# LariWa/Fractal-Image-Compression

Hardware: NVIDIA B200
Metric: encode_evals_per_s (higher is better)
Workload: dtype u8

## Files before the change

### fractal-image-compression_b200/csrc/fic_search_umma.cu

```cuda
#include <cuda_fp16.h>

#include <cmath>
#include <mutex>
#include <tuple>
#include <vector>

#include "fic_device.cuh"

namespace fic {

namespace {

constexpr int kTileN = 128;
constexpr int kBlockM = 128;
constexpr int kAccs = 4;
constexpr int kRowsPerSB = kBlockM * kAccs;
constexpr int kEpiWarps = 16;
constexpr int kThreads = (4 + kEpiWarps) * 32;
constexpr int kChunksPerTile = kTileN / 32;
constexpr int kBoundBytes = kChunksPerTile * 2 * 4 + 16 + kChunksPerTile * 4;
constexpr int kNormOff = kChunksPerTile * 2 * 4 + 16;
constexpr int kFlagLists = 2;
constexpr int kFlagCap = 32;
constexpr float kOneMinusEps = 1.0f - 1.9073486328125e-06f;
// ... 92 lines not shown
    static constexpr int A_SB_BYTES = C::NB * A_BLOCK_BYTES;
    static constexpr int KS0 = ksplit_p0<C>();
    static constexpr int SBO_B = KS0 * 256;
    static constexpr int SBO_P1 = (C::KS_B - KS0) * 256;
    static constexpr int B_OP_BYTES = (kTileN / 8) * SBO_B;
    static constexpr int P0_BYTES = B_OP_BYTES + kBoundBytes;
    static constexpr int P1_BYTES = (kTileN / 8) * SBO_P1;
    static constexpr int B_TILE_BYTES = P0_BYTES + P1_BYTES;
    static constexpr int SLOT_BYTES = C::KSPLIT ? ((P0_BYTES + 127) / 128) * 128 : B_TILE_BYTES;
    static constexpr int PAIR_P0_BYTES = B_OP_BYTES / 2, PAIR_P1_BYTES = P1_BYTES / 2;
    static constexpr int PAIR_SLOT_BYTES = PAIR_P0_BYTES > PAIR_P1_BYTES ? PAIR_P0_BYTES : PAIR_P1_BYTES;
    static constexpr int PAIR_STAGES = (C::NSTAGE * SLOT_BYTES) / PAIR_SLOT_BYTES < 12 ? (C::NSTAGE * SLOT_BYTES) / PAIR_SLOT_BYTES : 12;
    static constexpr int BAR_BYTES = 512;
    static constexpr int SMEM_BYTES = A_SB_BYTES + C::NSTAGE * SLOT_BYTES + 1024  + BAR_BYTES  +
                                      kRowsPerSB * 4 ;
};

__device__ __noinline__ float flag_threshold(float lb, float tie_abs)
{
    const float rad = lb * lb * kOneMinusEps - tie_abs;
    return rad > 0.0f ? sqrtf(rad) : -1.0f;
}

struct RowFilter { float thresh, lbmax; int cnt; };
__device__ __noinline__ RowFilter flag_chunk(RowFilter st, float lb, float ub, float tie_abs, int2 *list, int chunk_id,
                                             uint32_t sh_lb, int share)
{
    if (st.cnt < kFlagCap) list[st.cnt] = make_int2(chunk_id, __float_as_int(ub));
    st.cnt++;
    if (lb > st.lbmax) {
        st.lbmax = lb;
        if (share)
            asm volatile("red.shared.max.u32 [%0], %1;" ::"r"(sh_lb), "r"(__float_as_uint(lb)) : "memory");
        const float rad = lb * lb * kOneMinusEps - tie_abs;
        st.thresh = rad > 0.0f ? sqrtf(rad) : -1.0f;
    }
    return st;
}


__host__ __device__ __forceinline__ int64_t sweep_to_sorted(int64_t pos, uint32_t mult, int64_t nch)
{
    const uint64_t chunk = (uint64_t)pos >> 5;
    return (int64_t)(((chunk * (uint64_t)mult) % (uint64_t)nch) * 32 + ((uint64_t)pos & 31));
}

__global__ void k_umma_sortkeys(const int32_t *__restrict__ dsum, const int32_t *__restrict__ dsq, int n,
                                int64_t ND, uint32_t *__restrict__ keys, int32_t *__restrict__ vals)
{
    int64_t j = (int64_t)blockIdx.x * blockDim.x + threadIdx.x;
    if (j >= ND) return;
    int dmean;
    keys[j] = (uint32_t)dom_var(dsum[j], dsq[j], n, &dmean);
    vals[j] = (int32_t)j;
}


constexpr int kSortSub = 512;

__global__ void __launch_bounds__(256) k_sort_hist(const uint32_t *__restrict__ keys, int64_t n, int shift, int64_t nwarps,
                                                   uint32_t *__restrict__ hist)
{
    __shared__ uint32_t s_h[8][256];
    const int warp = threadIdx.x >> 5, lane = threadIdx.x & 31;
    const int64_t gw = (int64_t)blockIdx.x * 8 + warp;
    for (int d = lane; d < 256; d += 32) s_h[warp][d] = 0;
    __syncwarp();
    if (gw < nwarps) {
        const int64_t a = gw * kSortSub, b = a + kSortSub < n ? a + kSortSub : n;
        for (int64_t i = a + lane; i < b; i += 32) atomicAdd(&s_h[warp][(keys[i] >> shift) & 255u], 1u);
        __syncwarp();
        for (int d = lane; d < 256; d += 32) hist[(int64_t)d * nwarps + gw] = s_h[warp][d];
    }
}

__global__ void __launch_bounds__(256) k_sort_scan_rows(uint32_t *__restrict__ hist, int64_t nwarps, uint32_t *__restrict__ totals)
{
// ... 95 lines not shown
__device__ __forceinline__ uint32_t pack4(int a, int b, int c, int d)
{
    return (uint32_t)(a & 0xff) | ((uint32_t)(b & 0xff) << 8) | ((uint32_t)(c & 0xff) << 16) | ((uint32_t)(d & 0xff) << 24);
}

template <int n>
__host__ __device__ __forceinline__ int64_t raw_offset(int64_t pos, int c)
{
    return (pos >> 5) * (32 * n) + c * 512 + (pos & 31) * 16;
}

__device__ __forceinline__ uint32_t pack_h2(int lo, int hi)
{
    const __half2 v = __halves2half2(__int2half_rn(lo), __int2half_rn(hi));
    return *(const uint32_t *)&v;
}

template <int B, bool F16>
__global__ void __launch_bounds__(128)
k_umma_pack_domains(const uint8_t *__restrict__ dec, const int32_t *__restrict__ dsum,
                    const int32_t *__restrict__ dsq, const int32_t *__restrict__ perm, uint8_t *__restrict__ opB,
                    int32_t *__restrict__ pos_dom, int4 *__restrict__ pos_info,
                    uint8_t *__restrict__ pos_raw, int64_t *__restrict__ dom0_pos,
                    Geom g, int64_t ntiles, uint32_t mult)
{
    using L = Lay<B, F16>;
    constexpr int n = Cfg<B, F16>::n;
    const int64_t pos = (int64_t)blockIdx.x * blockDim.x + threadIdx.x;
    const int64_t tile = pos / kTileN;
    const int row = (int)(pos % kTileN);
    const int64_t sp = sweep_to_sorted(pos, mult, ntiles * kChunksPerTile);
    constexpr bool KSPLIT = Cfg<B, F16>::KSPLIT;
    uint8_t *blob = opB + tile * L::B_TILE_BYTES;
    uint8_t *rowp = blob + (row >> 3) * L::SBO_B + (row & 7) * 16;
    uint8_t *rowp1 = blob + L::P0_BYTES + (row >> 3) * L::SBO_P1 + (row & 7) * 16;
    constexpr int NCH = L::KS0 * 2;
    constexpr int NCH1 = (Cfg<B, F16>::KS_B - L::KS0) * 2;
    float rsd_hi = 0.0f, rsd_lo = __int_as_float(0x7f800000);
    int any_l = 0;
    if (sp >= g.ND) {
#pragma unroll
        for (int c = 0; c < NCH; c++) *(uint4 *)(rowp + c * 128) = make_uint4(0, 0, 0, 0);
#pragma unroll
        for (int c = 0; c < NCH1; c++) *(uint4 *)(rowp1 + c * 128) = make_uint4(0, 0, 0, 0);
        pos_dom[pos] = -1;
        pos_info[pos] = make_int4(-1, 0, 0, 0);
    } else {
        const int64_t j = perm[sp];
        const int gx = (int)(j % g.dpw), gy = (int)(j / g.dpw);
        const uint8_t *p = dec + (int64_t)(gy * g.step) * g.sw + gx * g.step;
        int dmean;
        const int varD = dom_var(dsum[j], dsq[j], n, &dmean);
        constexpr int PCH = n / 16;
        const int sgn = (!F16 && dmean == 0) ? -1 : 1;
// ... 43 lines not shown
                        hv[e] = max(-128, min(127, dv[w * 4 + e]));
                        lv[e] = dv[w * 4 + e] - hv[e];
                        any_l |= lv[e];
                    }
                    hw[w] = pack4(hv[0], hv[1], hv[2], hv[3]);
                    lw[w] = pack4(lv[0], lv[1], lv[2], lv[3]);
                }
                *(uint4 *)(rowp + c * 128) = make_uint4(hw[0], hw[1], hw[2], hw[3]);
                if (KSPLIT) *(uint4 *)(rowp1 + c * 128) = make_uint4(lw[0], lw[1], lw[2], lw[3]);
                else *(uint4 *)(rowp + (PCH + c) * 128) = make_uint4(lw[0], lw[1], lw[2], lw[3]);
            }
        }
        if (!F16) {
            const int alpha = sgn * (dsum[j] - n * dmean);
            const int a1 = alpha / 3, a2 = (alpha - a1) / 2, a3 = alpha - a1 - a2;
            constexpr int ACH = KSPLIT ? PCH : 2 * PCH;
            *(uint4 *)(rowp + ACH * 128) = make_uint4(
                (uint32_t)((-a1) & 0xff) | ((uint32_t)((-a2) & 0xff) << 8) | ((uint32_t)((-a3) & 0xff) << 16), 0, 0, 0);
            *(uint4 *)(rowp + (ACH + 1) * 128) = make_uint4(0, 0, 0, 0);
        }
        pos_dom[pos] = (int32_t)j;
        pos_info[pos] = make_int4((int32_t)j, varD, dsum[j], 0);
        if (j == 0) *dom0_pos = pos;
        if (varD > 0) {
            float r = __double2float_rn(__ddiv_rn(1.0, __dsqrt_rn((double)varD)));
            rsd_hi = r * (1.0f + 4.76837158203125e-07f);
            rsd_lo = r * (1.0f - 4.76837158203125e-07f);
        }
    }
    for (int o = 16; o > 0; o >>= 1) {
        rsd_hi = fmaxf(rsd_hi, __shfl_xor_sync(0xffffffffu, rsd_hi, o));
        rsd_lo = fminf(rsd_lo, __shfl_xor_sync(0xffffffffu, rsd_lo, o));
    }
    if ((threadIdx.x & 31) == 0) {
        if (rsd_hi == 0.0f) rsd_lo = 0.0f;
        *(float2 *)(blob + L::B_OP_BYTES + (row >> 5) * 8) = make_float2(rsd_hi, rsd_lo);
    }
    const int tile_has_l = __syncthreads_or(any_l != 0);
    if (threadIdx.x == 0) *(uint4 *)(blob + L::B_OP_BYTES + kChunksPerTile * 8) = make_uint4((uint32_t)tile_has_l, 0, 0, 0);
}

template <int B, bool F16>
__global__ void __launch_bounds__(128)
k_umma_pack_ranges(const uint8_t *__restrict__ src, const int32_t *__restrict__ rsum, uint8_t *__restrict__ opA,
                   int32_t *__restrict__ vRout, Geom g, int64_t j0, int64_t j1, int64_t rows_padded)
{
    using L = Lay<B, F16>;
    constexpr int n = Cfg<B, F16>::n;
    int64_t i = (int64_t)blockIdx.x * blockDim.x + threadIdx.x;
    if (i >= rows_padded) return;
    int64_t sb = i / L::ROWS_SB;
    int rr = (int)(i % L::ROWS_SB);
    int blk = rr / kBlockM, row = rr % kBlockM;
    uint8_t *rowp = opA + sb * L::A_SB_BYTES + blk * L::A_BLOCK_BYTES + (row >> 3) * L::SBO_A + (row & 7) * 16;
    constexpr int NCH = Cfg<B, F16>::KS_A * 2;
    const int64_t j = j0 + i / g.n_iso;
    const int kiso = (int)(i % g.n_iso);
    if (j >= j1) {
#pragma unroll
        for (int c = 0; c < NCH; c++) *(uint4 *)(rowp + c * 128) = make_uint4(0, 0, 0, 0);
        vRout[i] = 0;
        return;
    }
    int xr = (int)(j % g.rpw), yr = (int)(j / g.rpw);
    const uint8_t *p = src + (int64_t)(yr * B) * g.W + xr * B;
    int rmean;
    vRout[i] = centred_sum(rsum[j], n, &rmean);
    constexpr int PCH = n / 16;
#pragma unroll
    for (int c = 0; c < PCH; c++) {
        uint32_t w4[4];
#pragma unroll
        for (int w = 0; w < 4; w++) {
            int k = c * 16 + w * 4;
            if (kiso == 0) {
                w4[w] = *(const uint32_t *)(p + (int64_t)(k / B) * g.W + (k % B));
            } else {
                w4[w] = 0;
#pragma unroll
                for (int e = 0; e < 4; e++) {
                    int ry, rx;
                    iso_map(iso_inverse(kiso), B, (k + e) / B, (k + e) % B, &ry, &rx);
                    w4[w] |= (uint32_t)p[(int64_t)ry * g.W + rx] << (8 * e);
                }
            }
        }
        if (F16) {
            uint32_t hw[8];
#pragma unroll
            for (int w = 0; w < 4; w++) {
// ... 334 lines not shown
    asm("dp4a.u32.u32 %0, %1, %2, %3;" : "=r"(d) : "r"(a_u8x4), "r"(b_u8x4), "r"(c));
    return d;
}

__device__ __forceinline__ uint64_t make_desc(uint32_t saddr, uint32_t lbo_bytes, uint32_t sbo_bytes)
{
    return (uint64_t)((saddr >> 4) & 0x3fff) | ((uint64_t)((lbo_bytes >> 4) & 0x3fff) << 16) |
           ((uint64_t)((sbo_bytes >> 4) & 0x3fff) << 32) | ((uint64_t)1 << 46);
}

constexpr uint32_t kIdesc = (2u << 4) | (0u << 7) | (1u << 10) | ((uint32_t)(kTileN >> 3) << 17) |
                            ((uint32_t)(kBlockM >> 4) << 24);
constexpr uint32_t kIdescF16 = (1u << 4) | (0u << 7) | (0u << 10) | ((uint32_t)(kTileN >> 3) << 17) |
                               ((uint32_t)(kBlockM >> 4) << 24);
constexpr uint32_t kIdescPair = (2u << 4) | (0u << 7) | (1u << 10) | ((uint32_t)(kTileN >> 3) << 17) |
                                ((uint32_t)((2 * kBlockM) >> 4) << 24);
constexpr uint32_t kIdescF16Pair = (1u << 4) | (0u << 7) | (0u << 10) | ((uint32_t)(kTileN >> 3) << 17) |
                                   ((uint32_t)((2 * kBlockM) >> 4) << 24);


template <int B, bool F16, bool PAIR>
__host__ __device__ constexpr int epi_of() { return (!F16 || B == 16) ? 0 : ((B == 4 || PAIR) ? 3 : 2); }

template <int B, bool F16, bool PAIR, bool DUMP>
__global__ void __launch_bounds__(kThreads, 1)
k_umma_search(const uint8_t *__restrict__ opA, const uint8_t *__restrict__ opB, const int32_t *__restrict__ vRarr,
              const float *__restrict__ nRarr, int2 *__restrict__ flag_list, int32_t *__restrict__ flag_cnt, uint32_t *__restrict__ row_lb, int n_sb,
              int n_chunks, int ntiles, int iso_shift, int64_t rows_padded, int32_t *__restrict__ dump, int64_t dump_ld, volatile int *status)
{
    using C = Cfg<B, F16>;
    using L = Lay<B, F16>;
    static_assert(!PAIR || F16 || C::KSPLIT, "CTA pairs: kind::f16, or the K-split configurations (B = 16)");
    constexpr int EPI = DUMP ? 0 : epi_of<B, F16, PAIR>();
    constexpr int NISS = (PAIR && !C::KSPLIT) ? 2 : 1;
    constexpr int NSTAGE = PAIR ? L::PAIR_STAGES : C::NSTAGE;
    constexpr int SLOT = PAIR ? L::PAIR_SLOT_BYTES : L::SLOT_BYTES;
    extern __shared__ __align__(1024) uint8_t smem_raw[];
    uint8_t *smem = (uint8_t *)(((uintptr_t)smem_raw + 1023) & ~(uintptr_t)1023);
    uint8_t *sA = smem;
    uint8_t *sB = smem + L::A_SB_BYTES;
    uint64_t *bars = (uint64_t *)(sB + C::NSTAGE * L::SLOT_BYTES);
    uint32_t bar0 = smem_u32(bars);
    asm volatile("" : "+r"(bar0));
    auto BAR_B_FULL = [&](int s) { return bar0 + 8u * s; };
    auto BAR_B_EMPTY = [&](int s) { return bar0 + 8u * (NSTAGE + s); };
    auto BAR_T_FULL = [&](int q) { return bar0 + 8u * (2 * NSTAGE + q); };
    auto BAR_T_EMPTY = [&](int q) { return bar0 + 8u * (2 * NSTAGE + kAccs + q); };
    const uint32_t BAR_A_FULL = bar0 + 8u * (2 * NSTAGE + 2 * kAccs);
    const uint32_t BAR_A_EMPTY = BAR_A_FULL + 8u;
    uint32_t *tmem_slot = (uint32_t *)(bars + 2 * NSTAGE + 2 * kAccs + 2);
    const uint32_t s_has_l = bar0 + 400u;
    uint32_t *s_lb = (uint32_t *)((uint8_t *)bars + L::BAR_BYTES);

    const int warp = threadIdx.x >> 5, lane = threadIdx.x & 31;
    const uint32_t rank = PAIR ? cluster_ctarank() : 0u;
    const int u_first = PAIR ? (int)(blockIdx.x >> 1) : (int)blockIdx.x, u_step = PAIR ? (int)(gridDim.x >> 1) : (int)gridDim.x;
    const int n_sbu = PAIR ? (n_sb >> 1) : n_sb;

    if (warp == 1 && lane == 0) {
        const uint32_t both = (PAIR && rank == 0) ? 2u : 1u;
        for (int s = 0; s < NSTAGE; s++) {
            mbar_init(BAR_B_FULL(s), both);
            mbar_init(BAR_B_EMPTY(s), NISS);
        }
        for (int q = 0; q < kAccs; q++) {
            mbar_init(BAR_T_FULL(q), 1);
            mbar_init(BAR_T_EMPTY(q), both * (kEpiWarps / kAccs));
        }
        mbar_init(BAR_A_FULL, both);
        mbar_init(BAR_A_EMPTY, NISS);
        asm volatile("fence.mbarrier_init.release.cluster;" ::: "memory");
    }
    if (warp == 2) {
        if (PAIR) {
            asm volatile("tcgen05.alloc.cta_group::2.sync.aligned.shared::cta.b32 [%0], %1;" ::"r"(smem_u32(tmem_slot)), "r"(512u) : "memory");
            asm volatile("tcgen05.relinquish_alloc_permit.cta_group::2.sync.aligned;" ::: "memory");
        } else {
            asm volatile("tcgen05.alloc.cta_group::1.sync.aligned.shared::cta.b32 [%0], %1;" ::"r"(smem_u32(tmem_slot)), "r"(512u) : "memory");
            asm volatile("tcgen05.relinquish_alloc_permit.cta_group::1.sync.aligned;" ::: "memory");
        }
    }
    tc_fence_before();
    if (PAIR) cluster_sync_all();
    else __syncthreads();
    tc_fence_after();
    const uint32_t tmem_base = *tmem_slot;

    const int n_units = n_sbu * n_chunks;

    if (warp == 0) {
        if (lane == 0) {
            uint32_t stage = 0, phase = 0, a_phase = 0;
            for (int u = u_first; u < n_units; u += u_step) {
                int sb = PAIR ? 2 * (u % n_sbu) + (int)rank : u % n_sbu, ch = u / n_sbu;
                int t0 = (int)((int64_t)ch * ntiles / n_chunks), t1 = (int)((int64_t)(ch + 1) * ntiles / n_chunks);
                mbar_wait(BAR_A_EMPTY, a_phase ^ 1, status, 1);
                mbar_expect_tx(BAR_A_FULL, L::A_SB_BYTES);
                bulk_g2s(smem_u32(sA), opA + (int64_t)sb * L::A_SB_BYTES, L::A_SB_BYTES, BAR_A_FULL);
                for (int t = t0; t < t1; t++) {
                    const uint8_t *blob = opB + (int64_t)t * L::B_TILE_BYTES;
                    if (C::KSPLIT && PAIR) {
                        const uint32_t has_l = __ldg((const uint32_t *)(blob + L::B_OP_BYTES + kChunksPerTile * 8));
                        mbar_wait(BAR_B_EMPTY(stage), phase ^ 1, status, 2);
// ... 108 lines not shown
                        for (int t = t0; t < t1; t++) {
                            mbar_wait(BAR_B_FULL(stage), phase, status, 4);
                            const uint32_t has_l = lds_volatile_u32(s_has_l + 4u * stage);
                            mbar_arrive_cluster(mapa_u32(BAR_B_FULL(stage), 0));
                            if (++stage == NSTAGE) { stage = 0; phase ^= 1; }
                            if (has_l) {
                                mbar_wait(BAR_B_FULL(stage), phase, status, 4);
                                mbar_arrive_cluster(mapa_u32(BAR_B_FULL(stage), 0));
                                if (++stage == NSTAGE) { stage = 0; phase ^= 1; }
                            }
                        }
                        a_phase ^= 1;
                    }
                }
                __syncwarp();
            }
        } else if constexpr (PAIR) {
            if (rank == 0) {
                const int qi = warp >> 1;
                uint32_t stage = 0, phase = 0, a_phase = 0, t_phase = 0;
                const uint32_t elected = elect_one();
                const uint64_t a_desc0 = make_desc(smem_u32(sA), 128, L::SBO_A);
                const uint64_t b_desc0 = make_desc(smem_u32(sB), 128, L::SBO_B);
                for (int u = u_first; u < n_units; u += u_step) {
                    int ch = u / n_sbu;
                    int t0 = (int)((int64_t)ch * ntiles / n_chunks), t1 = (int)((int64_t)(ch + 1) * ntiles / n_chunks);
                    mbar_wait(BAR_A_FULL, a_phase, status, 3);
                    for (int t = t0; t < t1; t++) {
                        mbar_wait(BAR_B_FULL(stage), phase, status, 4);
                        tc_fence_after();
                        const uint64_t b_desc = b_desc0 + (uint64_t)((stage * SLOT) >> 4);
#pragma unroll
                        for (int k = 0; k < 2; k++) {
                            const int q = qi + 2 * k;
                            mbar_wait(BAR_T_EMPTY(q), ((t_phase >> k) & 1) ^ 1, status, 5);
                            tc_fence_after();
                            if (elected) {
#pragma unroll
                                for (int s = 0; s < C::NS; s++) {
                                    const uint64_t ad = a_desc0 + (uint64_t)((q * L::A_BLOCK_BYTES + C::amap(s) * 256) >> 4);
                                    tc_mma2_f16(tmem_base + q * kTileN, ad, b_desc + (uint64_t)((s * 256) >> 4), kIdescF16Pair, s > 0 ? 1u : 0u);
                                }
                                tc_commit2(BAR_T_FULL(q), 3u);
                                if (k == 1) tc_commit2(BAR_B_EMPTY(stage), 3u);
                            }
                            __syncwarp();
                            t_phase ^= 1u << k;
                        }
                        if (++stage == NSTAGE) { stage = 0; phase ^= 1; }
                    }
                    if (elected) tc_commit2(BAR_A_EMPTY, 3u);
                    __syncwarp();
                    a_phase ^= 1;
                }
            } else if (warp == 1) {
                if (lane == 0) {
                    uint32_t stage = 0, phase = 0, a_phase = 0;
                    const uint32_t ra_full = mapa_u32(BAR_A_FULL, 0);
                    for (int u = u_first; u < n_units; u += u_step) {
                        int ch = u / n_sbu;
                        int t0 = (int)((int64_t)ch * ntiles / n_chunks), t1 = (int)((int64_t)(ch + 1) * ntiles / n_chunks);
                        mbar_wait(BAR_A_FULL, a_phase, status, 3);
                        mbar_arrive_cluster(ra_full);
                        for (int t = t0; t < t1; t++) {
// ... 95 lines not shown
    } else if (warp >= 4) {
        const int e = warp - 4;
        const int lq = e & 3, q = e >> 2;
        const uint32_t ta = tmem_base + ((uint32_t)(lq * 32) << 16) + q * kTileN;
        uint32_t tf_phase = 0;
        const uint32_t bar_hand_back = PAIR ? mapa_u32(BAR_T_EMPTY(q), 0) : BAR_T_EMPTY(q);
        auto hand_back = [&]() {
            if (PAIR) mbar_arrive_cluster(bar_hand_back);
            else mbar_arrive(bar_hand_back);
        };
        constexpr bool SLACK = B == 16 && F16;
        const int n_units_mine = q < C::NB ? n_units : 0;
        for (int u = u_first; u < n_units_mine; u += u_step) {
            int sb = PAIR ? 2 * (u % n_sbu) + (int)rank : u % n_sbu, ch = u / n_sbu;
            int t0 = (int)((int64_t)ch * ntiles / n_chunks), t1 = (int)((int64_t)(ch + 1) * ntiles / n_chunks);
            const int64_t row = (int64_t)sb * L::ROWS_SB + q * kBlockM + lq * 32 + lane;
            const int vR = vRarr[row];
            const float nR = SLACK ? nRarr[row] : 0.0f;
            RowFilter st;
            st.thresh = (vR == 0) ? __int_as_float(0x7f800000) : -1.0f;
            st.lbmax = 0.0f;
            st.cnt = 0;
            const float tie_abs = (float)(vR * vR) * 4.76837158203125e-07f;
            const uint32_t sh_lb = smem_u32(s_lb + q * kBlockM + (((lq * 32 + lane) >> iso_shift) << iso_shift));
            if (iso_shift) {
                sts_u32(sh_lb, 0u);
                __syncwarp();
            }
            if (ch > 0 && vR != 0) {
                const float seed = __uint_as_float(*(volatile const uint32_t *)(row_lb + ((row >> iso_shift) << iso_shift)));
                if (seed > 0.0f) {
                    st.lbmax = seed;
                    st.thresh = flag_threshold(seed, tie_abs);
                }
            }
            int2 *const list0 = flag_list + (((int64_t)ch * rows_padded + row) * kFlagLists) * kFlagCap;
            int cnt0 = 0, cnt1 = 0;
            for (int t = t0; t < t1; t++) {
                const float4 *gb = (const float4 *)(opB + (int64_t)t * L::B_TILE_BYTES + L::B_OP_BYTES);
                const float4 bnd01 = __ldg(gb), bnd23 = __ldg(gb + 1);
                float4 bndn = make_float4(0.0f, 0.0f, 0.0f, 0.0f);
                if (SLACK) bndn = __ldg(gb + 3);
                mbar_wait(BAR_T_FULL(q), tf_phase, status, 7);
                tc_fence_after();
                if (iso_shift) {
                    const float other = __uint_as_float(lds_volatile_u32(sh_lb));
// ... 102 lines not shown
                        }
                    }
                    const float rhi = c == 0 ? bnd01.x : (c == 1 ? bnd01.z : (c == 2 ? bnd23.x : bnd23.z));
                    const float rlo = c == 0 ? bnd01.y : (c == 1 ? bnd01.w : (c == 2 ? bnd23.y : bnd23.w));
                    float Mu = M, Ml = M;
                    if (SLACK) {
                        const float pn = nR * (c == 0 ? bndn.x : (c == 1 ? bndn.y : (c == 2 ? bndn.z : bndn.w)));
                        if (pn >= 16777216.0f) {
                            const float sl = pn * 6.0e-5f;
                            Mu = M + sl;
                            Ml = fmaxf(M - sl, 0.0f);
                        }
                    }
                    const float ub = Mu * rhi;
                    if (ub > st.thresh) {
                        st.cnt = c < 2 ? cnt0 : cnt1;
                        st = flag_chunk(st, Ml * rlo, ub, tie_abs, list0 + (c >> 1) * kFlagCap, t * kChunksPerTile + c, sh_lb, iso_shift ? 1 : 0);
                        if (c < 2) cnt0 = st.cnt;
                        else cnt1 = st.cnt;
                    }
                }
                }
                tf_phase ^= 1;
            }
            flag_cnt[((int64_t)ch * rows_padded + row) * 2] = cnt0;
            flag_cnt[((int64_t)ch * rows_padded + row) * 2 + 1] = cnt1;
            if (st.lbmax > 0.0f) atomicMax(row_lb + ((row >> iso_shift) << iso_shift), __float_as_uint(st.lbmax));
        }
    }

    tc_fence_before();
    if (PAIR) cluster_sync_all();
    else __syncthreads();
    if (warp == 2) {
        tc_fence_after();
        if (PAIR) asm volatile("tcgen05.dealloc.cta_group::2.sync.aligned.b32 %0, %1;" ::"r"(tmem_base), "r"(512u) : "memory");
        else asm volatile("tcgen05.dealloc.cta_group::1.sync.aligned.b32 %0, %1;" ::"r"(tmem_base), "r"(512u) : "memory");
    }
}


template <bool F16, int N>
__global__ void __launch_bounds__(128, 1) k_mma_peak(int iters, uint32_t seed)
{
    extern __shared__ __align__(1024) uint8_t smem_raw[];
    uint8_t *smem = (uint8_t *)(((uintptr_t)smem_raw + 1023) & ~(uintptr_t)1023);
// ... 139 lines not shown
            const int cnt = __shfl_sync(0xffffffffu, my_cnt, lh);
            if (cnt == 0) continue;
            const int2 *lst = flag_list + (((int64_t)(lh / kFlagLists) * rows_padded + i) * kFlagLists + (lh % kFlagLists)) * kFlagCap;
            const int2 mine = lane < cnt ? lst[lane] : make_int2(0, 0);
            unsigned live = __ballot_sync(0xffffffffu, lane < cnt && __int_as_float(mine.y) > th);
            while (live) {
                const int e = __ffs(live) - 1;
                live &= live - 1;
                consider((int64_t)__shfl_sync(0xffffffffu, mine.x, e) * 32 + lane);
            }
        }
    } else {
        for (int64_t pos = lane; pos < npos; pos += 32) consider(pos);
    }
}

template <int B>
__global__ void __launch_bounds__(128)
k_umma_refine(const uint8_t *__restrict__ src, const int32_t *__restrict__ rsum, const uint8_t *__restrict__ pos_raw,
              const int4 *__restrict__ pos_info,
              const int2 *__restrict__ flag_list, const int32_t *__restrict__ flag_cnt,
              const uint32_t *__restrict__ row_lb, int n_chunks,
              int64_t rows_padded, int64_t rows, int64_t npos, const int64_t *__restrict__ dom0_pos,
              int32_t *__restrict__ best, Geom g, int64_t j0)
{
    constexpr int n = B * B;
    constexpr int NW = n / 4;
    const int warp = threadIdx.x >> 5, lane = threadIdx.x & 31;
    const int64_t i = (int64_t)blockIdx.x * 4 + warp;
    if (i >= rows) return;
    const int64_t j = j0 + i;
    int rmean;
    const int vR = centred_sum(rsum[j], n, &rmean);
    if (vR == 0) {
        if (lane == 0) best[j] = 0;
        return;
    }
    const int xr = (int)(j % g.rpw), yr = (int)(j / g.rpw);
    constexpr bool RW_SMEM = B == 16;
    __shared__ __align__(16) uint32_t s_rw[RW_SMEM ? 4 : 1][RW_SMEM ? NW : 4];
    __align__(16) uint32_t rw_reg[RW_SMEM ? 4 : NW];
    const uint32_t *rw;
    if constexpr (RW_SMEM) {
        for (int w = lane; w < NW; w += 32) {
            const int k = 4 * w;
            s_rw[warp][w] = __ldg((const uint32_t *)(src + (int64_t)(yr * B + k / B) * g.W + xr * B + (k % B)));
        }
        __syncwarp();
        rw = s_rw[warp];
    } else {
#pragma unroll
        for (int w = 0; w < NW; w++) {
            const int k = 4 * w;
            rw_reg[w] = __ldg((const uint32_t *)(src + (int64_t)(yr * B + k / B) * g.W + xr * B + (k % B)));
// ... 179 lines not shown
            const float vD = (float)pi.y;
            const float ax = pi.y > 0 ? __fdiv_rn(fabsf(kov), vD) : 0.0f;
            if (ax * (1.0f + 2.384185791015625e-07f) > th) {
                argmin_merge(be, bi, rgb_error(kov, vR, vD), idx);
                const float xlo = ax * (1.0f - 2.384185791015625e-07f);
                if (xlo > lb) { lb = xlo; th = flag_threshold(lb, tie_abs); }
            }
        }
    };
    if (lane == 0) consider(*dom0_pos);
    for_each_flagged(lane, i, rows_padded, n_chunks, npos, flag_list, flag_cnt, th_row, consider);
    warp_argmin(be, bi);
    if (lane == 0) best[j] = bi == 0x7fffffff ? 0 : bi;
}


inline int64_t pad_up(int64_t v, int64_t m) { return (v + m - 1) / m * m; }
inline uint64_t gcd_u64(uint64_t a, uint64_t b) { while (b) { uint64_t t = a % b; a = b; b = t; } return a; }

struct Plan {
    int64_t rp;
    int n_sb, ntiles, n_chunks;
    uint32_t mult;
    int64_t npos;
};

inline int rows_per_sb(const Geom &g) { return (g.C == 3 && g.B == 16 ? 2 : kAccs) * kBlockM; }

inline Plan make_plan(const Geom &g, int64_t rows, int num_sms)
{
    Plan p;
    const int rows_sb = rows_per_sb(g);
    p.rp = pad_up(rows, 2 * rows_sb);
    p.n_sb = (int)(p.rp / rows_sb);
    p.ntiles = (int)((g.ND + kTileN - 1) / kTileN);
    p.npos = (int64_t)p.ntiles * kTileN;
    p.n_chunks = 1;
    const double tile_s = (g.B == 16 ? (g.C == 3 ? 2300.0 : 4650.0) : (g.B == 8 ? 1550.0 : 1400.0)) / 1.9e9;
    const double flag_s = 0.11e-9 * (g.n / 64.0) * (g.n > 64 ? 0.7 : 1.0);
    double best_cost = 0;
    for (int c = 1; c <= 8 && c <= p.ntiles; c++) {
        const int64_t units = (int64_t)p.n_sb * c;
        const int64_t waves = (units + num_sms - 1) / num_sms;
        const double tiles_per_unit = (double)((p.ntiles + c - 1) / c);
        const double flags_per_row = 2.0 * (log(2.0 * tiles_per_unit) + 0.58) + 2.0 * (c - 1) * 1.5;
        const double cost = (double)waves * tiles_per_unit * tile_s + (double)rows * flags_per_row * flag_s;
        if (c == 1 || cost < best_cost * 0.98) { best_cost = cost; p.n_chunks = c; }
    }
    const uint64_t nch = (uint64_t)p.ntiles * kChunksPerTile;
    uint64_t m = (uint64_t)((double)nch * 0.6180339887498949) | 1u;
    while (gcd_u64(m, nch) != 1) m += 2;
    p.mult = nch <= 8 ? 1u : (uint32_t)(m % nch);
    return p;
}

template <int B, bool F16>
struct OpBLayout {
    size_t off_posdom, off_posinfo, off_posraw, off_dom0, off_keys0, off_keys1, off_vals0, off_vals1, off_temp,
        temp_bytes, total;
    OpBLayout(const Geom &g, const Plan &p)
    {
        size_t o = (size_t)p.ntiles * Lay<B, F16>::B_TILE_BYTES;
        auto take = [&](size_t bytes) { size_t at = (o + 255) & ~(size_t)255; o = at + bytes; return at; };
        off_posdom = take((size_t)p.npos * 4);
        off_posinfo = take((size_t)p.npos * 16);
        off_posraw = take((size_t)p.npos * (B * B));
        off_dom0 = take(16);
        off_keys0 = take((size_t)g.ND * 4);
        off_keys1 = take((size_t)g.ND * 4);
        off_vals0 = take((size_t)g.ND * 4);
        off_vals1 = take((size_t)g.ND * 4);
        temp_bytes = sort_hist_bytes(g.ND);
        off_temp = take(temp_bytes + 256);
        total = o + 256;
    }
};

template <int B, bool F16>
struct OpALayout {
    static constexpr int kCntSlots = 4;
    size_t off_vR, off_cnt, off_list, off_lb, off_norm, total;
    explicit OpALayout(const Plan &p)
    {
        off_vR = (size_t)p.n_sb * Lay<B, F16>::A_SB_BYTES;
        off_cnt = off_vR + (size_t)p.rp * 4;
        off_list = off_cnt + (size_t)p.rp * p.n_chunks * kCntSlots * 4;
        off_lb = off_list + (size_t)p.rp * p.n_chunks * kFlagLists * kFlagCap * sizeof(int2);
        off_norm = off_lb + (size_t)p.rp * 4;
        total = off_norm + (size_t)p.rp * 4 + 1024;
    }
};

template <int B, bool F16>
size_t opA_bytes_t(const Geom &g, int64_t rows, int num_sms)
{
    return OpALayout<B, F16>(make_plan(g, rows, num_sms)).total;
}

using KernelT = void (*)(const uint8_t *, const uint8_t *, const int32_t *, const float *, int2 *, int32_t *, uint32_t *, int, int,
                         int, int, int64_t, int32_t *, int64_t, volatile int *);

template <int B, bool F16>
constexpr bool pair_capable() { return F16 || B == 16; }
template <int B, bool F16>
constexpr bool pair_default() { return pair_capable<B, F16>() && B >= 8; }

inline bool pair_launchable(KernelT kern, int smem_bytes)
{
    static std::mutex mu;
    static std::vector<std::tuple<KernelT, int, bool>> known;
    int dev = 0;
    cudaGetDevice(&dev);
// ... 31 lines not shown
             cudaEvent_t k0, cudaEvent_t k1, int pair_mode, int *pair_used, int32_t *dump, int64_t dump_ld, int *status_dev)
{
    using L = Lay<B, F16>;
    if (j1 <= j0) return 0;
    const int64_t rows = (j1 - j0) * g.n_iso;
    Plan p = make_plan(g, rows, num_sms);
    const int64_t rp = p.rp;
    uint8_t *opA = w.opA;
    const OpALayout<B, F16> la(p);
    int32_t *vR = (int32_t *)(opA + la.off_vR);
    int32_t *flag_cnt = (int32_t *)(opA + la.off_cnt);
    int2 *flag_list = (int2 *)(opA + la.off_list);
    uint32_t *row_lb = (uint32_t *)(opA + la.off_lb);
    float *row_norm = (float *)(opA + la.off_norm);
    const bool rgb = g.C == 3;
    if (rgb && !F16) { *err = "the RGB tensor path is kind::f16 only"; return -1; }
    OpBLayout<B, F16> lay(g, p);
    int32_t *pos_dom = (int32_t *)(w.opB + lay.off_posdom);
    int4 *pos_info = (int4 *)(w.opB + lay.off_posinfo);
    uint8_t *pos_raw = w.opB + lay.off_posraw;
    int64_t *dom0 = (int64_t *)(w.opB + lay.off_dom0);
    int launches = 0;
    cudaError_t ce;
    uint32_t *keys0 = (uint32_t *)(w.opB + lay.off_keys0), *keys1 = (uint32_t *)(w.opB + lay.off_keys1);
    int32_t *vals0 = (int32_t *)(w.opB + lay.off_vals0), *vals1 = (int32_t *)(w.opB + lay.off_vals1);
    if (rgb) k_umma_sortkeys_rgb<<<(unsigned)((g.ND + 255) / 256), 256, 0, s>>>(w.dsum, g.n, g.ND, keys0, vals0);
    else k_umma_sortkeys<<<(unsigned)((g.ND + 255) / 256), 256, 0, s>>>(w.dsum, w.dsq, g.n, g.ND, keys0, vals0);
    launches += 1 + launch_sort_pairs(keys0, vals0, keys1, vals1, (uint32_t *)(w.opB + lay.off_temp), g.ND, s);
    const int32_t *perm = vals1;
    if constexpr (F16) {
        if (rgb) {
            launches += launch_sum_planes(w.dec, w.dec3, g, s);
            k_umma_pack_domains_rgb<B><<<(unsigned)((p.npos + 127) / 128), 128, 0, s>>>(
                w.dec3, w.dsum, perm, w.opB, pos_dom, pos_info, dom0, g, p.ntiles, p.mult);
            k_umma_pack_ranges_rgb<B><<<(unsigned)((rp + 127) / 128), 128, 0, s>>>(w.src, w.rsum, opA, vR, B == 16 ? row_norm : nullptr, g, j0, j1, rp);
        }
    }
    if (!rgb) {
        k_umma_pack_domains<B, F16><<<(unsigned)((p.npos + 127) / 128), 128, 0, s>>>(
            w.dec, w.dsum, w.dsq, perm, w.opB, pos_dom, pos_info, pos_raw, dom0, g, p.ntiles, p.mult);
        k_umma_pack_ranges<B, F16><<<(unsigned)((rp + 127) / 128), 128, 0, s>>>(w.src, w.rsum, opA, vR, g, j0, j1, rp);
    }
    launches += 2;
    bool pair = false;
    KernelT kern = dump ? k_umma_search<B, F16, false, true> : k_umma_search<B, F16, false, false>;
    if constexpr (pair_capable<B, F16>()) {
        pair = (pair_mode == FIC_UMMA_PAIR_ON || (pair_mode != FIC_UMMA_PAIR_OFF && pair_default<B, F16>())) && num_sms >= 2;
        if (pair) {
            KernelT pk = dump ? k_umma_search<B, F16, true, true> : k_umma_search<B, F16, true, false>;
            ce = cudaFuncSetAttribute(pk, cudaFuncAttributeMaxDynamicSharedMemorySize, L::SMEM_BYTES);
            if (ce != cudaSuccess) { *err = cudaGetErrorString(ce); return -1; }
            if (pair_launchable(pk, L::SMEM_BYTES)) kern = pk;
            else pair = false;
        }
    }
    if (pair_used) *pair_used = pair ? 1 : 0;
    ce = cudaFuncSetAttribute(kern, cudaFuncAttributeMaxDynamicSharedMemorySize, L::SMEM_BYTES);
    if (ce != cudaSuccess) { *err = cudaGetErrorString(ce); return -1; }
    int n_units = pair ? (p.n_sb / 2) * p.n_chunks : p.n_sb * p.n_chunks;
    const int slots = pair ? num_sms / 2 : num_sms;
    int grid = (n_units < slots ? n_units : slots) * (pair ? 2 : 1);
    if (k0) cudaEventRecord(k0, s);
    cudaMemsetAsync(row_lb, 0, (size_t)rp * 4, s);
    {
        cudaLaunchConfig_t cfg = {};
        cfg.gridDim = dim3((unsigned)grid);
        cfg.blockDim = dim3(kThreads);
        cfg.dynamicSmemBytes = L::SMEM_BYTES;
        cfg.stream = s;
        cudaLaunchAttribute at[1];
        at[0].id = cudaLaunchAttributeClusterDimension;
        at[0].val.clusterDim.x = 2;
        at[0].val.clusterDim.y = 1;
        at[0].val.clusterDim.z = 1;
        cfg.attrs = at;
        cfg.numAttrs = pair ? 1 : 0;
        const uint8_t *opA_c = opA, *opB_c = w.opB;
        const int32_t *vR_c = vR;
        const float *norm_c = row_norm;
        const int iso_shift = g.n_iso > 1 ? 3 : 0;
        volatile int *status_v = status_dev;
        ce = cudaLaunchKernelEx(&cfg, kern, opA_c, opB_c, vR_c, norm_c, flag_list, flag_cnt, row_lb, p.n_sb, p.n_chunks, p.ntiles, iso_shift,
                                rp, dump, dump_ld, status_v);
        if (ce != cudaSuccess) { *err = cudaGetErrorString(ce); return -1; }
    }
    if (k1) cudaEventRecord(k1, s);
    if (rgb) {
        if constexpr (F16)
            k_umma_refine_rgb<B><<<(unsigned)((rows + 3) / 4), 128, 0, s>>>(w.src, w.rsum, w.opB, pos_info, flag_list, flag_cnt,
                                                                            row_lb, p.n_chunks, rp, rows, p.npos, dom0, w.best, g, j0);
    } else if (g.n_iso > 1)
        k_umma_refine_iso<B><<<(unsigned)((j1 - j0 + 3) / 4), 128, 0, s>>>(w.src, w.rsum, pos_raw, pos_info, flag_list, flag_cnt,
                                                                         row_lb, p.n_chunks, rp, j1 - j0, p.npos, dom0, w.best, g, j0);
    else
        k_umma_refine<B><<<(unsigned)((rows + 3) / 4), 128, 0, s>>>(w.src, w.rsum, pos_raw, pos_info, flag_list, flag_cnt,
                                                                    row_lb, p.n_chunks, rp, rows, p.npos, dom0, w.best, g, j0);
    launches += 2;
    ce = cudaGetLastError();
    if (ce != cudaSuccess) { *err = cudaGetErrorString(ce); return -1; }
    return launches;
}

#define FIC_UMMA_DISPATCH(B_, F_, EXPR_I8_4, EXPR_I8_8, EXPR_I8_16, EXPR_F16_4, EXPR_F16_8, EXPR_F16_16) \
    ((B_) == 16 ? ((F_) ? (EXPR_F16_16) : (EXPR_I8_16)) : ((F_) ? ((B_) == 8 ? (EXPR_F16_8) : (EXPR_F16_4)) : ((B_) == 8 ? (EXPR_I8_8) : (EXPR_I8_4))))

}

int umma_default_kind(const Geom &g) { return g.B == 16 ? FIC_UMMA_KIND_I8 : FIC_UMMA_KIND_F16; }

static bool use_f16(const Geom &g, int kind)
{
    if (g.C == 3) return true;
    if (g.B == 16) return false;
    return (kind == FIC_UMMA_KIND_AUTO ? umma_default_kind(g) : kind) == FIC_UMMA_KIND_F16;
}

void umma_debug_positions(const Work &w, const Geom &g, int64_t rows, int num_sms, int kind, const int32_t **d_pos_dom,
                          int64_t *npos)
{
// ... 243 lines not shown
```

Measured before the change: 13390.

## Prune domain tiles by angular bounds between range and domain blocks

Adds angular pruning for the B=8 f16 pair search. Domains are sorted by variance plus an angle bin, and ranges are sorted by their angle. Each domain tile stores its angle interval, and the epilogue warps publish per-row-block angle windows derived from the current best threshold through cluster shared memory. The MMA warp then skips the full MMA chain for tiles that fall outside the window, issuing a single zero MMA instead. This cuts tensor-core and epilogue work but adds sorting, per-block theta computation, extra kernels and cross-warp window traffic, and it depends on the angular bound being conservative to keep results exact.

```diff
diff --git a/fractal-image-compression_b200/csrc/fic_search_umma.cu b/fractal-image-compression_b200/csrc/fic_search_umma.cu
--- a/fractal-image-compression_b200/csrc/fic_search_umma.cu
+++ b/fractal-image-compression_b200/csrc/fic_search_umma.cu
@@ -138,6 +138,19 @@
     return rad > 0.0f ? sqrtf(rad) : -1.0f;
 }
 
+constexpr float kAngSlack = 1.0e-5f;
+constexpr float kAngQ = 4095.0f / 1.5707963267948966f;
+constexpr int kPruneBins = 16;
+
+__host__ __device__ inline double block_theta(long long pu, long long pv, long long sq)
+{
+    const double p2 = ((double)pu * (double)pu + (double)pv * (double)pv) / 1344.0;
+    const double q2 = (double)sq - p2;
+    return atan2(sqrt(q2 > 0.0 ? q2 : 0.0), sqrt(p2));
+}
+__device__ __forceinline__ uint32_t ang_lo(float th) { return (uint32_t)fminf(4095.0f, fmaxf(0.0f, floorf((th - kAngSlack) * kAngQ))); }
+__device__ __forceinline__ uint32_t ang_hi(float th) { return (uint32_t)fminf(4095.0f, fmaxf(0.0f, ceilf((th + kAngSlack) * kAngQ))); }
+
 struct RowFilter { float thresh, lbmax; int cnt; };
 __device__ __noinline__ RowFilter flag_chunk(RowFilter st, float lb, float ub, float tie_abs, int2 *list, int chunk_id,
                                              uint32_t sh_lb, int share)
@@ -161,14 +174,48 @@
     return (int64_t)(((chunk * (uint64_t)mult) % (uint64_t)nch) * 32 + ((uint64_t)pos & 31));
 }
 
+__device__ __forceinline__ double block8_theta(const uint8_t *__restrict__ p, int64_t stride, int mean)
+{
+    long long pu = 0, pv = 0, sq = 0;
+    for (int y = 0; y < 8; y++)
+        for (int x = 0; x < 8; x++) {
+            const int a = (int)p[y * stride + x] - mean;
+            pu += a * (2 * x - 7);
+            pv += a * (2 * y - 7);
+            sq += a * a;
+        }
+    return block_theta(pu, pv, sq);
+}
+
 __global__ void k_umma_sortkeys(const int32_t *__restrict__ dsum, const int32_t *__restrict__ dsq, int n,
-                                int64_t ND, uint32_t *__restrict__ keys, int32_t *__restrict__ vals)
+                                int64_t ND, uint32_t *__restrict__ keys, int32_t *__restrict__ vals,
+                                const uint8_t *__restrict__ dec, Geom g, int prune)
 {
     int64_t j = (int64_t)blockIdx.x * blockDim.x + threadIdx.x;
     if (j >= ND) return;
     int dmean;
-    keys[j] = (uint32_t)dom_var(dsum[j], dsq[j], n, &dmean);
+    uint32_t key = (uint32_t)dom_var(dsum[j], dsq[j], n, &dmean);
+    if (prune) {
+        const int gx = (int)(j % g.dpw), gy = (int)(j / g.dpw);
+        const double th = block8_theta(dec + (int64_t)(gy * g.step) * g.sw + gx * g.step, g.sw, dmean);
+        key |= (uint32_t)min(kPruneBins - 1, (int)(th * (kPruneBins / 1.5707963267948966))) << 20;
+    }
+    keys[j] = key;
     vals[j] = (int32_t)j;
+}
+
+__global__ void k_umma_rangekeys(const uint8_t *__restrict__ src, const int32_t *__restrict__ rsum, Geom g, int64_t j0,
+                                 int64_t rows, uint32_t *__restrict__ keys, int32_t *__restrict__ vals)
+{
+    int64_t i = (int64_t)blockIdx.x * blockDim.x + threadIdx.x;
+    if (i >= rows) return;
+    const int64_t j = j0 + i;
+    const int xr = (int)(j % g.rpw), yr = (int)(j / g.rpw);
+    int rmean;
+    centred_sum(rsum[j], 64, &rmean);
+    const double th = block8_theta(src + (int64_t)(yr * 8) * g.W + xr * 8, g.W, rmean);
+    keys[i] = (uint32_t)min(16777215.0, th * (16777215.0 / 1.5707963267948966));
+    vals[i] = (int32_t)i;
 }
 
 
@@ -310,14 +357,16 @@
                     const int32_t *__restrict__ dsq, const int32_t *__restrict__ perm, uint8_t *__restrict__ opB,
                     int32_t *__restrict__ pos_dom, int4 *__restrict__ pos_info,
                     uint8_t *__restrict__ pos_raw, int64_t *__restrict__ dom0_pos,
-                    Geom g, int64_t ntiles, uint32_t mult)
+                    Geom g, int64_t ntiles, uint32_t mult, uint32_t tmult)
 {
     using L = Lay<B, F16>;
     constexpr int n = Cfg<B, F16>::n;
     const int64_t pos = (int64_t)blockIdx.x * blockDim.x + threadIdx.x;
     const int64_t tile = pos / kTileN;
     const int row = (int)(pos % kTileN);
-    const int64_t sp = sweep_to_sorted(pos, mult, ntiles * kChunksPerTile);
+    const int64_t sp = tmult ? (int64_t)(((uint64_t)tile * tmult) % (uint64_t)ntiles) * kTileN + row
+                             : sweep_to_sorted(pos, mult, ntiles * kChunksPerTile);
+    uint32_t th_lo = 4095u, th_hi = 0u;
     constexpr bool KSPLIT = Cfg<B, F16>::KSPLIT;
     uint8_t *blob = opB + tile * L::B_TILE_BYTES;
     uint8_t *rowp = blob + (row >> 3) * L::SBO_B + (row & 7) * 16;
@@ -407,6 +456,11 @@
         pos_dom[pos] = (int32_t)j;
         pos_info[pos] = make_int4((int32_t)j, varD, dsum[j], 0);
         if (j == 0) *dom0_pos = pos;
+        if (B == 8 && tmult) {
+            const float th = (float)block8_theta(p, g.sw, dmean);
+            th_lo = ang_lo(th);
+            th_hi = ang_hi(th);
+        }
         if (varD > 0) {
             float r = __double2float_rn(__ddiv_rn(1.0, __dsqrt_rn((double)varD)));
             rsd_hi = r * (1.0f + 4.76837158203125e-07f);
@@ -421,14 +475,20 @@
         if (rsd_hi == 0.0f) rsd_lo = 0.0f;
         *(float2 *)(blob + L::B_OP_BYTES + (row >> 5) * 8) = make_float2(rsd_hi, rsd_lo);
     }
+    __shared__ uint32_t s_lo, s_hi;
+    if (threadIdx.x == 0) { s_lo = 4095u; s_hi = 0u; }
+    __syncthreads();
+    if (tmult) { atomicMin(&s_lo, th_lo); atomicMax(&s_hi, th_hi); }
     const int tile_has_l = __syncthreads_or(any_l != 0);
-    if (threadIdx.x == 0) *(uint4 *)(blob + L::B_OP_BYTES + kChunksPerTile * 8) = make_uint4((uint32_t)tile_has_l, 0, 0, 0);
+    if (threadIdx.x == 0)
+        *(uint4 *)(blob + L::B_OP_BYTES + kChunksPerTile * 8) = make_uint4((uint32_t)tile_has_l, s_lo | (s_hi << 12), 0, 0);
 }
 
 template <int B, bool F16>
 __global__ void __launch_bounds__(128)
 k_umma_pack_ranges(const uint8_t *__restrict__ src, const int32_t *__restrict__ rsum, uint8_t *__restrict__ opA,
-                   int32_t *__restrict__ vRout, Geom g, int64_t j0, int64_t j1, int64_t rows_padded)
+                   int32_t *__restrict__ vRout, Geom g, int64_t j0, int64_t j1, int64_t rows_padded,
+                   const int32_t *__restrict__ rmap, float2 *__restrict__ rgeo)
 {
     using L = Lay<B, F16>;
     constexpr int n = Cfg<B, F16>::n;
@@ -439,7 +499,7 @@
     int blk = rr / kBlockM, row = rr % kBlockM;
     uint8_t *rowp = opA + sb * L::A_SB_BYTES + blk * L::A_BLOCK_BYTES + (row >> 3) * L::SBO_A + (row & 7) * 16;
     constexpr int NCH = Cfg<B, F16>::KS_A * 2;
-    const int64_t j = j0 + i / g.n_iso;
+    const int64_t j = j0 + (rmap && i < j1 - j0 ? (int64_t)rmap[i] : i / g.n_iso);
     const int kiso = (int)(i % g.n_iso);
     if (j >= j1) {
 #pragma unroll
@@ -451,6 +511,15 @@
     const uint8_t *p = src + (int64_t)(yr * B) * g.W + xr * B;
     int rmean;
     vRout[i] = centred_sum(rsum[j], n, &rmean);
+    if (B == 8 && rgeo) {
+        long long sq = 0;
+        for (int y = 0; y < 8; y++)
+            for (int x = 0; x < 8; x++) {
+                const int a = (int)p[(int64_t)y * g.W + x] - rmean;
+                sq += a * a;
+            }
+        rgeo[i] = make_float2((float)block8_theta(p, g.W, rmean), (float)sqrt((double)sq) * (1.0f + 4.76837158203125e-07f));
+    }
     constexpr int PCH = n / 16;
 #pragma unroll
     for (int c = 0; c < PCH; c++) {
@@ -831,7 +900,7 @@
 template <int B, bool F16, bool PAIR>
 __host__ __device__ constexpr int epi_of() { return (!F16 || B == 16) ? 0 : ((B == 4 || PAIR) ? 3 : 2); }
 
-template <int B, bool F16, bool PAIR, bool DUMP>
+template <int B, bool F16, bool PAIR, bool DUMP, bool PRUNE = false>
 __global__ void __launch_bounds__(kThreads, 1)
 k_umma_search(const uint8_t *__restrict__ opA, const uint8_t *__restrict__ opB, const int32_t *__restrict__ vRarr,
               const float *__restrict__ nRarr, int2 *__restrict__ flag_list, int32_t *__restrict__ flag_cnt, uint32_t *__restrict__ row_lb, int n_sb,
@@ -840,6 +909,7 @@
     using C = Cfg<B, F16>;
     using L = Lay<B, F16>;
     static_assert(!PAIR || F16 || C::KSPLIT, "CTA pairs: kind::f16, or the K-split configurations (B = 16)");
+    static_assert(!PRUNE || (PAIR && F16 && B == 8 && !DUMP), "pruning: the B = 8 kind::f16 pair kernel");
     constexpr int EPI = DUMP ? 0 : epi_of<B, F16, PAIR>();
     constexpr int NISS = (PAIR && !C::KSPLIT) ? 2 : 1;
     constexpr int NSTAGE = PAIR ? L::PAIR_STAGES : C::NSTAGE;
@@ -860,6 +930,7 @@
     uint32_t *tmem_slot = (uint32_t *)(bars + 2 * NSTAGE + 2 * kAccs + 2);
     const uint32_t s_has_l = bar0 + 400u;
     uint32_t *s_lb = (uint32_t *)((uint8_t *)bars + L::BAR_BYTES);
+    const uint32_t s_win = bar0 + 288u;
 
     const int warp = threadIdx.x >> 5, lane = threadIdx.x & 31;
     const uint32_t rank = PAIR ? cluster_ctarank() : 0u;
@@ -888,6 +959,11 @@
             asm volatile("tcgen05.alloc.cta_group::1.sync.aligned.shared::cta.b32 [%0], %1;" ::"r"(smem_u32(tmem_slot)), "r"(512u) : "memory");
             asm volatile("tcgen05.relinquish_alloc_permit.cta_group::1.sync.aligned;" ::: "memory");
         }
+    }
+    if constexpr (PRUNE) {
+        for (int k = threadIdx.x; k < kRowsPerSB; k += kThreads) s_lb[k] = 0u;
+        if (threadIdx.x < 32) sts_u32(s_win + 4u * threadIdx.x, 0u);
+        asm volatile("fence.proxy.async.shared::cta;" ::: "memory");
     }
     tc_fence_before();
     if (PAIR) cluster_sync_all();
@@ -1042,11 +1118,29 @@
                 const uint32_t elected = elect_one();
                 const uint64_t a_desc0 = make_desc(smem_u32(sA), 128, L::SBO_A);
                 const uint64_t b_desc0 = make_desc(smem_u32(sB), 128, L::SBO_B);
+                const uint64_t z_desc = make_desc(smem_u32(s_lb), 128, 256);
+                uint32_t wlo[2] = {0u, 0u}, whi[2] = {4095u, 4095u};
                 for (int u = u_first; u < n_units; u += u_step) {
                     int ch = u / n_sbu;
                     int t0 = (int)((int64_t)ch * ntiles / n_chunks), t1 = (int)((int64_t)(ch + 1) * ntiles / n_chunks);
+                    const uint32_t tag = (uint32_t)(((u - u_first) / u_step) & 0x7f) + 1u;
                     mbar_wait(BAR_A_FULL, a_phase, status, 3);
                     for (int t = t0; t < t1; t++) {
+                        uint32_t tw = 0u;
+                        if constexpr (PRUNE) {
+                            tw = __ldg((const uint32_t *)(opB + (int64_t)t * L::B_TILE_BYTES + L::B_OP_BYTES + kChunksPerTile * 8 + 4));
+                            if (((t - t0) & 7) == 0) {
+#pragma unroll
+                                for (int k = 0; k < 2; k++) {
+                                    const uint32_t wd = lane < 8 ? lds_volatile_u32(s_win + 4u * ((qi + 2 * k) * 8 + lane)) : 0u;
+                                    const bool ok = __all_sync(0xffffffffu, lane >= 8 || (wd >> 24) == tag);
+                                    const uint32_t lo = __reduce_min_sync(0xffffffffu, lane < 8 ? wd & 0xfffu : 4095u);
+                                    const uint32_t hi = __reduce_max_sync(0xffffffffu, lane < 8 ? (wd >> 12) & 0xfffu : 0u);
+                                    wlo[k] = ok ? lo : 0u;
+                                    whi[k] = ok ? hi : 4095u;
+                                }
+                            }
+                        }
                         mbar_wait(BAR_B_FULL(stage), phase, status, 4);
                         tc_fence_after();
                         const uint64_t b_desc = b_desc0 + (uint64_t)((stage * SLOT) >> 4);
@@ -1055,11 +1149,16 @@
                             const int q = qi + 2 * k;
                             mbar_wait(BAR_T_EMPTY(q), ((t_phase >> k) & 1) ^ 1, status, 5);
                             tc_fence_after();
+                            const bool skip = PRUNE && ((tw >> 12) < wlo[k] || (tw & 0xfffu) > whi[k] || wlo[k] > whi[k]);
                             if (elected) {
-#pragma unroll
-                                for (int s = 0; s < C::NS; s++) {
-                                    const uint64_t ad = a_desc0 + (uint64_t)((q * L::A_BLOCK_BYTES + C::amap(s) * 256) >> 4);
-                                    tc_mma2_f16(tmem_base + q * kTileN, ad, b_desc + (uint64_t)((s * 256) >> 4), kIdescF16Pair, s > 0 ? 1u : 0u);
+                                if (skip) {
+                                    tc_mma2_f16(tmem_base + q * kTileN, a_desc0 + (uint64_t)((q * L::A_BLOCK_BYTES) >> 4), z_desc, kIdescF16Pair, 0u);
+                                } else {
+#pragma unroll
+                                    for (int s = 0; s < C::NS; s++) {
+                                        const uint64_t ad = a_desc0 + (uint64_t)((q * L::A_BLOCK_BYTES + C::amap(s) * 256) >> 4);
+                                        tc_mma2_f16(tmem_base + q * kTileN, ad, b_desc + (uint64_t)((s * 256) >> 4), kIdescF16Pair, s > 0 ? 1u : 0u);
+                                    }
                                 }
                                 tc_commit2(BAR_T_FULL(q), 3u);
                                 if (k == 1) tc_commit2(BAR_B_EMPTY(stage), 3u);
@@ -1201,6 +1300,9 @@
             st.lbmax = 0.0f;
             st.cnt = 0;
             const float tie_abs = (float)(vR * vR) * 4.76837158203125e-07f;
+            float2 geo = make_float2(0.0f, 0.0f);
+            if constexpr (PRUNE) geo = ((const float2 *)nRarr)[row];
+            const uint32_t tag = (uint32_t)(((u - u_first) / u_step) & 0x7f) + 1u;
             const uint32_t sh_lb = smem_u32(s_lb + q * kBlockM + (((lq * 32 + lane) >> iso_shift) << iso_shift));
             if (iso_shift) {
                 sts_u32(sh_lb, 0u);
@@ -1349,6 +1451,28 @@
                 }
                 }
                 tf_phase ^= 1;
+                if constexpr (PRUNE) {
+                    if (((t - t0) & 7) == 7) {
+                        uint32_t lo = 4095u, hi = 0u;
+                        if (vR != 0) {
+                            if (st.thresh < 0.0f) {
+                                lo = 0u;
+                                hi = 4095u;
+                            } else {
+                                const float ratio = st.thresh / geo.y * (1.0f - 3.814697265625e-06f);
+                                const float phi = ratio >= 1.0f ? 0.0f : acosf(ratio) + kAngSlack;
+                                lo = ang_lo(geo.x - phi);
+                                hi = ang_hi(geo.x + phi);
+                            }
+                        }
+                        lo = __reduce_min_sync(0xffffffffu, lo);
+                        hi = __reduce_max_sync(0xffffffffu, hi);
+                        if (lane == 0) {
+                            const uint32_t dst = mapa_u32(s_win + 4u * (q * 8 + (int)rank * 4 + lq), 0);
+                            asm volatile("st.shared::cluster.u32 [%0], %1;" ::"r"(dst), "r"((tag << 24) | lo | (hi << 12)) : "memory");
+                        }
+                    }
+                }
             }
             flag_cnt[((int64_t)ch * rows_padded + row) * 2] = cnt0;
             flag_cnt[((int64_t)ch * rows_padded + row) * 2 + 1] = cnt1;
@@ -1534,14 +1658,14 @@
               const int2 *__restrict__ flag_list, const int32_t *__restrict__ flag_cnt,
               const uint32_t *__restrict__ row_lb, int n_chunks,
               int64_t rows_padded, int64_t rows, int64_t npos, const int64_t *__restrict__ dom0_pos,
-              int32_t *__restrict__ best, Geom g, int64_t j0)
+              int32_t *__restrict__ best, Geom g, int64_t j0, const int32_t *__restrict__ rmap)
 {
     constexpr int n = B * B;
     constexpr int NW = n / 4;
     const int warp = threadIdx.x >> 5, lane = threadIdx.x & 31;
     const int64_t i = (int64_t)blockIdx.x * 4 + warp;
     if (i >= rows) return;
-    const int64_t j = j0 + i;
+    const int64_t j = j0 + (rmap ? (int64_t)rmap[i] : i);
     int rmean;
     const int vR = centred_sum(rsum[j], n, &rmean);
     if (vR == 0) {
@@ -1767,6 +1891,7 @@
     int64_t rp;
     int n_sb, ntiles, n_chunks;
     uint32_t mult;
+    uint32_t tmult;
     int64_t npos;
 };
 
@@ -1796,6 +1921,10 @@
     uint64_t m = (uint64_t)((double)nch * 0.6180339887498949) | 1u;
     while (gcd_u64(m, nch) != 1) m += 2;
     p.mult = nch <= 8 ? 1u : (uint32_t)(m % nch);
+    const uint64_t nt = (uint64_t)p.ntiles;
+    uint64_t tm = (uint64_t)((double)nt * 0.6180339887498949) | 1u;
+    while (gcd_u64(tm, nt) != 1) tm += 2;
+    p.tmult = nt <= 8 ? 1u : (uint32_t)(tm % nt);
     return p;
 }
 
@@ -1824,7 +1953,7 @@
 template <int B, bool F16>
 struct OpALayout {
     static constexpr int kCntSlots = 4;
-    size_t off_vR, off_cnt, off_list, off_lb, off_norm, total;
+    size_t off_vR, off_cnt, off_list, off_lb, off_norm, off_rmap, off_geo, total;
     explicit OpALayout(const Plan &p)
     {
         off_vR = (size_t)p.n_sb * Lay<B, F16>::A_SB_BYTES;
@@ -1832,7 +1961,9 @@
         off_list = off_cnt + (size_t)p.rp * p.n_chunks * kCntSlots * 4;
         off_lb = off_list + (size_t)p.rp * p.n_chunks * kFlagLists * kFlagCap * sizeof(int2);
         off_norm = off_lb + (size_t)p.rp * 4;
-        total = off_norm + (size_t)p.rp * 4 + 1024;
+        off_rmap = off_norm + (size_t)p.rp * 4;
+        off_geo = off_rmap + (size_t)p.rp * 4;
+        total = off_geo + (size_t)p.rp * 8 + 1024;
     }
 };
 
@@ -1910,26 +2041,6 @@
     int64_t *dom0 = (int64_t *)(w.opB + lay.off_dom0);
     int launches = 0;
     cudaError_t ce;
-    uint32_t *keys0 = (uint32_t *)(w.opB + lay.off_keys0), *keys1 = (uint32_t *)(w.opB + lay.off_keys1);
-    int32_t *vals0 = (int32_t *)(w.opB + lay.off_vals0), *vals1 = (int32_t *)(w.opB + lay.off_vals1);
-    if (rgb) k_umma_sortkeys_rgb<<<(unsigned)((g.ND + 255) / 256), 256, 0, s>>>(w.dsum, g.n, g.ND, keys0, vals0);
-    else k_umma_sortkeys<<<(unsigned)((g.ND + 255) / 256), 256, 0, s>>>(w.dsum, w.dsq, g.n, g.ND, keys0, vals0);
-    launches += 1 + launch_sort_pairs(keys0, vals0, keys1, vals1, (uint32_t *)(w.opB + lay.off_temp), g.ND, s);
-    const int32_t *perm = vals1;
-    if constexpr (F16) {
-        if (rgb) {
-            launches += launch_sum_planes(w.dec, w.dec3, g, s);
-            k_umma_pack_domains_rgb<B><<<(unsigned)((p.npos + 127) / 128), 128, 0, s>>>(
-                w.dec3, w.dsum, perm, w.opB, pos_dom, pos_info, dom0, g, p.ntiles, p.mult);
-            k_umma_pack_ranges_rgb<B><<<(unsigned)((rp + 127) / 128), 128, 0, s>>>(w.src, w.rsum, opA, vR, B == 16 ? row_norm : nullptr, g, j0, j1, rp);
-        }
-    }
-    if (!rgb) {
-        k_umma_pack_domains<B, F16><<<(unsigned)((p.npos + 127) / 128), 128, 0, s>>>(
-            w.dec, w.dsum, w.dsq, perm, w.opB, pos_dom, pos_info, pos_raw, dom0, g, p.ntiles, p.mult);
-        k_umma_pack_ranges<B, F16><<<(unsigned)((rp + 127) / 128), 128, 0, s>>>(w.src, w.rsum, opA, vR, g, j0, j1, rp);
-    }
-    launches += 2;
     bool pair = false;
     KernelT kern = dump ? k_umma_search<B, F16, false, true> : k_umma_search<B, F16, false, false>;
     if constexpr (pair_capable<B, F16>()) {
@@ -1942,6 +2053,42 @@
             else pair = false;
         }
     }
+    bool prune = false;
+    if constexpr (B == 8 && F16) {
+        prune = pair && !rgb && g.n_iso == 1 && !dump && rows <= g.ND;
+        if (prune) {
+            kern = k_umma_search<8, true, true, false, true>;
+            ce = cudaFuncSetAttribute(kern, cudaFuncAttributeMaxDynamicSharedMemorySize, L::SMEM_BYTES);
+            if (ce != cudaSuccess) { *err = cudaGetErrorString(ce); return -1; }
+        }
+    }
+    int32_t *rmap = prune ? (int32_t *)(opA + la.off_rmap) : nullptr;
+    float2 *rgeo = prune ? (float2 *)(opA + la.off_geo) : nullptr;
+    uint32_t *keys0 = (uint32_t *)(w.opB + lay.off_keys0), *keys1 = (uint32_t *)(w.opB + lay.off_keys1);
+    int32_t *vals0 = (int32_t *)(w.opB + lay.off_vals0), *vals1 = (int32_t *)(w.opB + lay.off_vals1);
+    if (prune) {
+        k_umma_rangekeys<<<(unsigned)((rows + 255) / 256), 256, 0, s>>>(w.src, w.rsum, g, j0, rows, keys0, vals0);
+        launches += 1 + launch_sort_pairs(keys0, vals0, keys1, vals1, (uint32_t *)(w.opB + lay.off_temp), rows, s);
+        cudaMemcpyAsync(rmap, vals1, (size_t)rows * 4, cudaMemcpyDeviceToDevice, s);
+    }
+    if (rgb) k_umma_sortkeys_rgb<<<(unsigned)((g.ND + 255) / 256), 256, 0, s>>>(w.dsum, g.n, g.ND, keys0, vals0);
+    else k_umma_sortkeys<<<(unsigned)((g.ND + 255) / 256), 256, 0, s>>>(w.dsum, w.dsq, g.n, g.ND, keys0, vals0, w.dec, g, prune ? 1 : 0);
+    launches += 1 + launch_sort_pairs(keys0, vals0, keys1, vals1, (uint32_t *)(w.opB + lay.off_temp), g.ND, s);
+    const int32_t *perm = vals1;
+    if constexpr (F16) {
+        if (rgb) {
+            launches += launch_sum_planes(w.dec, w.dec3, g, s);
+            k_umma_pack_domains_rgb<B><<<(unsigned)((p.npos + 127) / 128), 128, 0, s>>>(
+                w.dec3, w.dsum, perm, w.opB, pos_dom, pos_info, dom0, g, p.ntiles, p.mult);
+            k_umma_pack_ranges_rgb<B><<<(unsigned)((rp + 127) / 128), 128, 0, s>>>(w.src, w.rsum, opA, vR, B == 16 ? row_norm : nullptr, g, j0, j1, rp);
+        }
+    }
+    if (!rgb) {
+        k_umma_pack_domains<B, F16><<<(unsigned)((p.npos + 127) / 128), 128, 0, s>>>(
+            w.dec, w.dsum, w.dsq, perm, w.opB, pos_dom, pos_info, pos_raw, dom0, g, p.ntiles, p.mult, prune ? p.tmult : 0u);
+        k_umma_pack_ranges<B, F16><<<(unsigned)((rp + 127) / 128), 128, 0, s>>>(w.src, w.rsum, opA, vR, g, j0, j1, rp, rmap, rgeo);
+    }
+    launches += 2;
     if (pair_used) *pair_used = pair ? 1 : 0;
     ce = cudaFuncSetAttribute(kern, cudaFuncAttributeMaxDynamicSharedMemorySize, L::SMEM_BYTES);
     if (ce != cudaSuccess) { *err = cudaGetErrorString(ce); return -1; }
@@ -1965,7 +2112,7 @@
         cfg.numAttrs = pair ? 1 : 0;
         const uint8_t *opA_c = opA, *opB_c = w.opB;
         const int32_t *vR_c = vR;
-        const float *norm_c = row_norm;
+        const float *norm_c = prune ? (const float *)rgeo : row_norm;
         const int iso_shift = g.n_iso > 1 ? 3 : 0;
         volatile int *status_v = status_dev;
         ce = cudaLaunchKernelEx(&cfg, kern, opA_c, opB_c, vR_c, norm_c, flag_list, flag_cnt, row_lb, p.n_sb, p.n_chunks, p.ntiles, iso_shift,
@@ -1982,7 +2129,7 @@
                                                                          row_lb, p.n_chunks, rp, j1 - j0, p.npos, dom0, w.best, g, j0);
     else
         k_umma_refine<B><<<(unsigned)((rows + 3) / 4), 128, 0, s>>>(w.src, w.rsum, pos_raw, pos_info, flag_list, flag_cnt,
-                                                                    row_lb, p.n_chunks, rp, rows, p.npos, dom0, w.best, g, j0);
+                                                                    row_lb, p.n_chunks, rp, rows, p.npos, dom0, w.best, g, j0, rmap);
     launches += 2;
     ce = cudaGetLastError();
     if (ce != cudaSuccess) { *err = cudaGetErrorString(ce); return -1; }
```

Result: slower. 5320 (median of 6 runs) (-60.3%).
